# Gyeeta/gyeeta

Hardware: AMD Instinct MI355X
Metric: events/sec ingested + p50/p99 quantile error vs reference, 1→8 MI355X (higher is better)
Workload: dtype int64; 1 GPU; C3/C4: 10000 hosts x 1000 services, raw 24-B tcp_ipv4_resp_event_t stream, uniform over services, 1 window (ingest + window close) per step; service_keys_total=10000000, multi_level_windows=0, td_pend_cap=1920, td_pend_cap_is_library_default=False, exchange=none, exchange_requested=none, exchange_fallback=False

## Files before the change

gyeeta_amd/csrc/gys_kernels.hpp:

```cpp
#pragma once

#include "gys_device.hpp"

namespace gys {

#define GYS_HUGE_VALUE_BITS 20
#define GYS_HUGE_BINS (1u << GYS_HUGE_VALUE_BITS)
#define GYS_ROW_BITS 6
#define GYS_ROW_MASK 0x3Fu
#define GYS_ROW_V6 0x20u
#define GYS_BM_WORDS 32u
#define GYS_STAGED_WORD(tresp, cli_port) ((uint64_t)(((uint32_t)(tresp) << GYS_ROW_BITS) | ((uint32_t)(cli_port) & 0x1Fu)))
#define GYS_STAGED_WORD_FAM(tresp, cli_port, v6) ((uint32_t)(((uint32_t)(tresp) << GYS_ROW_BITS) | ((v6) ? GYS_ROW_V6 : 0u) | ((uint32_t)(cli_port) & 0x1Fu)))

enum { CTR_RESP_EVENTS = 0, CTR_RESP_DROP_RANGE, CTR_RESP_DROP_NOLISTENER, CTR_CONN_EVENTS, CTR_CONN_UNKNOWN, CTR_LSTATE_RECORDS,
       CTR_LSTATE_MISSED, CTR_LSTATE_ERRORS, CTR_LSTATE_DELETED, CTR_TD_MERGES, CTR_TD_MERGE_VALUES, CTR_ACTCONN_RECORDS, CTR_ACTCONN_REMOTE_LISTEN, CTR_ACTCONN_UNKNOWN,
       CTR_CONN_NEW, CTR_CONN_CLOSED, CTR_CONN_CLOSED_NO_NOTIFY, CTR_CONN_CLI_SIDE, CTR_RESP_RUN_OVERFLOW, CTR_NUM };

__global__ void k_table_set(DevTable t, const uint64_t *kv, uint32_t n)
{
	const uint32_t i = blockIdx.x * blockDim.x + threadIdx.x;
	if (i >= n) return;
	const uint64_t key = kv[2u * i];
	uint32_t h = get_uint64_hash(key) & t.mask;
// ... 1622 lines not shown
		for (uint32_t i = tid; i < GYS_IVL; i += NT) {
			s_icnt[i] = 0;
			s_imin[i] = 0xFFFFFFFFu;
			s_imax[i] = 0;
			s_clt[i] = 0;
		}
		if (tid < 16u) {
			s_fa[tid] = 0;
			s_fw[tid] = 0;
			s_fbm[tid] = 0;
			s_fbm[tid + 16u] = 0;
		}
		if (tid == 0) {
			s_fmm[0] = INT32_MAX;
			s_fmm[1] = INT32_MIN;
			s_fmm[2] = INT32_MIN;
		}
		__syncthreads();
		if (c0) {
			s_thr[pos0] = ceil_div_sum_cnt(sm0, c0);
			s_cpfx[pos0] = e0;
		}
		if (tid == 0) s_cpfx[nc] = nold;
		__syncthreads();
		{
			const uint32_t *pend = p.td_pend + (size_t)slot * p.pcap;
			int32_t lmin = INT32_MAX, lmax = INT32_MIN, wmax = INT32_MIN;
			for (uint32_t i = tid; i < m; i += NT) {
				const uint32_t word = i < ent.nbuf ? pend[i] : p.staged[run0 + (i - ent.nbuf)];
				const uint32_t uv = word >> GYS_ROW_BITS;
				uint32_t lo = 0;
#pragma unroll
				for (uint32_t step = GYS_NBP / 2; step >= 1u; step >>= 1)
					if (s_thr[lo + step - 1u] <= uv) lo += step;
				const uint32_t iv = lo + value_grid(uv);
				s_x[i] = (iv << 20) | uv;
				atomicAdd(&s_icnt[iv], 1u);
				atomicMin(&s_imin[iv], uv);
				atomicMax(&s_imax[iv], uv);
				atomicAdd(&s_clt[lo + 1], 1u);
				if (i >= nh) {
					const uint32_t b = resp_bucket((int64_t)uv);
					const unsigned long long one = GYS_PACK_ONE | (unsigned long long)uv;
					atomicAdd(&s_fa[b], one);
					lmin = min(lmin, (int32_t)uv);
					lmax = max(lmax, (int32_t)uv);
					if (i >= nwin0) {
						atomicAdd(&s_fw[b], one);
						const uint32_t r = word & GYS_ROW_MASK;
						atomicOr(&s_fbm[r >> 1], (1u << b) << ((r & 1u) * 16u));
						wmax = max(wmax, (int32_t)uv);
					}
				}
			}
			if (!query && m > nh) {
				lmin = wave_min_i32(lmin);
				lmax = wave_max_i32(lmax);
				wmax = wave_max_i32(wmax);
				if (lane == 0) {
					if (lmin != INT32_MAX) atomicMin(&s_fmm[0], lmin);
					if (lmax != INT32_MIN) atomicMax(&s_fmm[1], lmax);
					if (wmax != INT32_MIN) atomicMax(&s_fmm[2], wmax);
				}
			}
		}
		__syncthreads();
		if (wave == 0) {
			uint32_t t[5], gcl[5];
			uint32_t own = 0, gown = 0;
#pragma unroll
			for (int k = 0; k < 5; ++k) {
				t[k] = s_icnt[5u * lane + k];
				gcl[k] = s_clt[5u * lane + k];
				own += t[k];
				gown += gcl[k];
			}
			const uint32_t inc = wave_incl_scan_u32(own), ginc = wave_incl_scan_u32(gown);
			uint32_t ex = inc - own, gex = ginc - gown;
#pragma unroll
			for (int k = 0; k < 5; ++k) {
				s_ioff[5u * lane + k] = ex;
				s_icnt[5u * lane + k] = ex;
				ex += t[k];
				gex += gcl[k];
				s_clt[5u * lane + k] = gex;
			}
			if (lane == 63u) s_ioff[GYS_IVL] = inc;
		}
		__syncthreads();
		for (uint32_t i = tid; i < m; i += NT) {
			const uint32_t x = s_x[i];
			s_g[atomicAdd(&s_icnt[x >> 20], 1u)] = x;
		}
		__syncthreads();
		if (c0) {
			const uint64_t mid2 = 2ull * (e0 + (uint64_t)s_clt[pos0 + 1]) + (uint64_t)c0;
			uint32_t a = 0;
#pragma unroll
			for (uint32_t step = GYS_NBP / 2; step >= 1u; step >>= 1)
				if (mid2 >= s_T[a + step]) a += step;
			atomicAdd(&s_osum[a], (unsigned long long)sm0);
			atomicAdd(&s_ocnt[a], c0);
		}
		for (uint32_t e = tid; e < m; e += NT) {
			const uint32_t x = s_g[e];
			const uint32_t iv = x >> 20;
			uint32_t r = e;
			if (s_imin[iv] != s_imax[iv]) {
				const uint32_t gb = s_ioff[iv], ge = s_ioff[iv + 1];
				r = gb;
				for (uint32_t t = gb; t < ge; ++t) {
					const uint32_t y = s_g[t];
					r += (y < x || (y == x && t < e)) ? 1u : 0u;
				}
			}
			const uint64_t mid2 = 2ull * ((uint64_t)r + s_cpfx[iv - value_grid(x & 0xFFFFFu)]) + 1ull;
			uint32_t a = 0;
#pragma unroll
			for (uint32_t step = GYS_NBP / 2; step >= 1u; step >>= 1)
				if (mid2 >= s_T[a + step]) a += step;
			atomicAdd(&s_osum[a], (unsigned long long)(x & 0xFFFFFu));
			atomicAdd(&s_ocnt[a], 1u);
		}
		__syncthreads();
		if (tid < GYS_TD_NB) {
			int64_t *ws = query ? q.out_sum + (size_t)w * GYS_TD_NB : p.td_sum + (size_t)slot * GYS_TD_NB;
			uint32_t *wc = query ? q.out_cnt + (size_t)w * GYS_TD_NB : p.td_cnt + (size_t)slot * GYS_TD_NB;
			ws[tid] = (int64_t)s_osum[tid];
			wc[tid] = s_ocnt[tid];
		}
		if (!query) {
			const uint32_t n_all = m - nh, n_win = m > nwin0 ? m - nwin0 : 0u;
			if (tid < 16u && n_all) fold_records(p, slot, tid, mt.w != mt.z, s_fa[tid], s_fw[tid], n_all, n_win, s_fmm[1], s_fmm[2], s_fbm[tid], s_fbm[tid + 16u]);
			if (tid == 16u) {
				*(uint4 *)&p.td_meta[slot] = make_uint4(0u, 0u, mt.z, n_win ? mt.z : mt.w);
				p.td_cur[slot] = 0;
				if (n_all) {
					const int2 mm = p.td_minmax[slot];
					if (s_fmm[0] < mm.x || s_fmm[1] > mm.y) p.td_minmax[slot] = make_int2(min(mm.x, s_fmm[0]), max(mm.y, s_fmm[1]));
				}
			}
		}
		__syncthreads();
	}
}

#ifndef GYS_MB_SKIP
#define GYS_MB_SKIP 0
#endif
#define GYS_MB_EXACT 1024u
#define GYS_MB_BINS 2048u
#define GYS_MB_BPT 8u

__device__ __forceinline__ uint32_t mb_bin(uint32_t v)
{
	if (v < GYS_MB_EXACT) return v;
	const uint32_t msb = 31u - (uint32_t)__clz((int)v);
	return GYS_MB_EXACT + (msb - 10u) * 64u + ((v >> (msb - 6u)) & 63u);
}

struct MergeBP {
	DigestP d;
	const MergeEnt *list;
	const uint32_t *count;
	int64_t *out_sum;
	uint32_t *out_cnt;
	MergeEnt *slow_list;
	uint32_t *slow_count;
	const double *qs;
	uint32_t nq;
	double *qout;
};

__device__ __forceinline__ double td_quantile_dev(const uint32_t *c_cnt, const unsigned long long *c_sum, const uint32_t *c_wb, uint32_t nc, uint32_t N,
						  int32_t vmin, int32_t vmax, double q)
{
	if (!N) return 0.0;
	if (q < 0.0) q = 0.0;
	if (q > 1.0) q = 1.0;
	const double t = q * (double)N;
	uint32_t lo = 0, hi = nc;
	while (lo < hi) {
		const uint32_t mid = (lo + hi) >> 1;
		if (t < (double)c_wb[mid] + (double)c_cnt[mid] * 0.5) hi = mid; else lo = mid + 1;
	}
	double res;
	if (lo < nc) {
		const double mean = (double)(int64_t)c_sum[lo] / (double)c_cnt[lo];
		const double c = (double)c_wb[lo] + (double)c_cnt[lo] * 0.5;
		if (lo == 0) {
			const double l = (double)vmin;
			res = c <= 0.0 ? mean : l + (mean - l) * (t / c);
		} else {
			const double pm = (double)(int64_t)c_sum[lo - 1] / (double)c_cnt[lo - 1];
			const double pc = (double)c_wb[lo - 1] + (double)c_cnt[lo - 1] * 0.5;
			res = pm + (mean - pm) * ((t - pc) / (c - pc));
		}
	} else {
		const double pm = (double)(int64_t)c_sum[nc - 1] / (double)c_cnt[nc - 1];
		const double pc = (double)c_wb[nc - 1] + (double)c_cnt[nc - 1] * 0.5;
		const double h = (double)vmax, span = (double)N - pc;
		res = span <= 0.0 ? h : pm + (h - pm) * ((t - pc) / span);
	}
	return floor(res + 0.5);
}

#define GYS_MB_BIG_CAP 1024u
#ifndef GYS_MB_WAVES16
#define GYS_MB_WAVES16 5
#endif
template <bool SCAN, uint32_t VPT = 4u>
__global__ __launch_bounds__(256, (VPT == 16u ? GYS_MB_WAVES16 : 8)) void k_digest_bins(MergeBP q_arg)
{
#if defined(__HIP_DEVICE_COMPILE__)
	typedef const MergeBP __attribute__((address_space(4))) *KernargP;
	KernargP q_k = (KernargP)__builtin_amdgcn_kernarg_segment_ptr();
#define GYS_MB_Q_RELOAD() asm volatile("" : "+s"(q_k))
	const MergeBP &q = *(const MergeBP *)q_k;
#else
#define GYS_MB_Q_RELOAD() (void)0
	const MergeBP &q = q_arg;
#endif
	const DigestP &p = q.d;
	static_assert(VPT == 4u || VPT == 8u || VPT == 16u || VPT == 64u, "merges of 1024 / 2048 / 4096 values; 64: up to 16 384, streamed");
	constexpr bool STREAM = VPT > 16u;
	constexpr uint32_t RV = STREAM ? 8u : VPT;
	__shared__ __align__(16) uint32_t s_bin[GYS_MB_BINS];
	constexpr uint32_t BIG_CAP = GYS_MB_BIG_CAP;
	__shared__ uint32_t s_big[BIG_CAP];
	__shared__ uint32_t s_thr[GYS_NBP];
	__shared__ uint32_t s_cpfx[GYS_NBP + 1];
	__shared__ uint32_t s_T[GYS_NBP];
	__shared__ unsigned long long s_osum[GYS_TD_NB];
	__shared__ uint32_t s_ocnt[GYS_TD_NB];
	__shared__ unsigned long long s_oval[GYS_TD_NB];
	__shared__ unsigned long long s_fa[16], s_fw[16];
	__shared__ uint32_t s_fbm[GYS_BM_WORDS];
	__shared__ int32_t s_fmm[3];
	__shared__ uint32_t s_wv[4], s_ws[4], s_nbig;
	__shared__ uint64_t s_ww[4];
	const uint32_t nent = SCAN ? p.nsvc : *q.count;
	const bool query = SCAN || q.out_sum != nullptr;
	uint32_t bk_first = 0, bk_chg = GYS_MB_BPT;
	if (GYS_MB_BPT * threadIdx.x < GYS_MB_EXACT) {
		bk_first = resp_bucket((int64_t)(GYS_MB_BPT * threadIdx.x));
		for (uint32_t k = GYS_MB_BPT - 1u; k >= 1u; --k)
			if (resp_bucket((int64_t)(GYS_MB_BPT * threadIdx.x + k)) != bk_first) bk_chg = k;
	}

	for (uint32_t w = blockIdx.x; w < nent; w += gridDim.x) {
		uint32_t tid = threadIdx.x;
		GYS_OPAQUE_VGPR(tid);
		GYS_MB_Q_RELOAD();
		const uint32_t lane = tid & 63u, wave = tid >> 6;
		MergeEnt ent;
		if (SCAN) ent = MergeEnt{w, min(p.td_meta[w].npend, p.pend_cap), 0u, 0u};
		else ent = q.list[w];
		const uint32_t m = ent.nbuf + ent.mrun;
		if (m > 256u * VPT) continue;
		const uint32_t slot = ent.slot;
		const uint4 mt = *(const uint4 *)&p.td_meta[slot];
		const uint32_t nh = query ? m : (mt.y & 0xFFFFu), nw = mt.y >> 16;
		const uint32_t nh_mm = SCAN ? (mt.y & 0xFFFFu) : nh;
		const uint32_t nwin0 = max(nh, nw);
		const uint32_t run0 = ent.off_end - ent.mrun;
		uint32_t c0 = 0;
		int64_t sm0 = 0;
		if (tid < GYS_TD_NB) {
			c0 = p.td_cnt[(size_t)slot * GYS_TD_NB + tid];
			sm0 = p.td_sum[(size_t)slot * GYS_TD_NB + tid];
		}
		uint32_t wd[RV];
		const uint32_t *const pend = p.td_pend + (size_t)slot * p.pcap;
		{
#pragma unroll
			for (uint32_t k = 0; k < RV; ++k) {
				const uint32_t i = tid + 256u * k;
				wd[k] = 0;
				if (i < m) wd[k] = i < ent.nbuf ? pend[i] : p.staged[run0 + (i - ent.nbuf)];
			}
		}
		if (GYS_MB_SKIP & 32) {
			uint32_t x = c0 ^ (uint32_t)sm0;
#pragma unroll
			for (uint32_t k = 0; k < RV; ++k) x ^= wd[k];
			if (x == 0xDEADBEEFu) p.td_cur[slot] = 1;
			continue;
		}
		if (m == 0 && !SCAN) {
			if (query && tid < GYS_TD_NB) {
				q.out_sum[(size_t)w * GYS_TD_NB + tid] = sm0;
				q.out_cnt[(size_t)w * GYS_TD_NB + tid] = c0;
			}
			continue;
		}
#pragma unroll
		for (uint32_t k = 0; k < GYS_MB_BPT; ++k) s_bin[tid + 256u * k] = 0;
		s_thr[tid] = 0xFFFFFFFFu;
		if (tid < GYS_TD_NB) {
			s_osum[tid] = 0;
			s_ocnt[tid] = 0;
			s_oval[tid] = 0;
		}
		if (tid < 16u) {
			s_fa[tid] = 0;
			s_fw[tid] = 0;
			s_fbm[tid] = 0;
			s_fbm[tid + 16u] = 0;
		}
		if (tid == 0) {
			s_fmm[0] = INT32_MAX;
			s_fmm[1] = INT32_MIN;
			s_fmm[2] = INT32_MIN;
			s_nbig = 0;
		}
		const unsigned long long b0 = __ballot(c0 != 0);
		const uint64_t inc = wave_incl_scan_u64(c0);
		if (lane == 63u) s_ww[wave] = inc;
		if (lane == 0u) s_wv[wave] = (uint32_t)__popcll(b0);
		__syncthreads();
		uint32_t pbase = 0, nc = 0;
		uint64_t wbase = 0, nold64 = 0;
#pragma unroll
		for (uint32_t k = 0; k < 4u; ++k) {
			if (k < wave) {
				pbase += s_wv[k];
				wbase += s_ww[k];
			}
			nc += s_wv[k];
			nold64 += s_ww[k];
		}
		if (nold64 + (uint64_t)m >= (1ull << 31)) {
			if (tid == 0) q.slow_list[atomicAdd(q.slow_count, 1u)] = ent;
			__syncthreads();
			continue;
		}
		if (SCAN && m == 0) {
			if (tid < GYS_TD_NB) {
				s_osum[tid] = (unsigned long long)sm0;
				s_ocnt[tid] = c0;
			}
			__syncthreads();
		} else {
		const uint32_t pos0 = pbase + (uint32_t)__popcll(b0 & (lane ? (~0ull >> (64 - lane)) : 0ull));
		const uint32_t e0 = (uint32_t)(wbase + inc - c0), nold = (uint32_t)nold64;
		const uint32_t twoN = 2u * (nold + m);
		uint32_t thr = 0;
		if (c0) {
			thr = ceil_div_sum_cnt(sm0, c0);
			s_thr[pos0] = thr;
			s_cpfx[pos0] = e0;
			atomicAdd(&s_bin[mb_bin(thr)], 1u << 16);
		}
		if (tid == 0) s_cpfx[nc] = nold;
		s_T[tid] = (tid >= 1u && tid < GYS_TD_NB) ? (uint32_t)td_threshold(c_td_bnd[tid], (uint64_t)twoN) : (tid ? 0xFFFFFFFFu : 0u);
		const bool fold_scan = !query && nh == 0u;
		int32_t lmin = INT32_MAX, lmax = INT32_MIN, wmax = INT32_MIN;
		for (uint32_t cb = 0; cb < (STREAM ? m : 1u); cb += 256u * RV) {
		if (STREAM && cb) {
#pragma unroll
			for (uint32_t k = 0; k < RV; ++k) {
				const uint32_t i = cb + tid + 256u * k;
				wd[k] = 0;
				if (i < m) wd[k] = i < ent.nbuf ? pend[i] : p.staged[run0 + (i - ent.nbuf)];
			}
		}
#pragma unroll
		for (uint32_t k = 0; k < RV; ++k) {
			const uint32_t i = cb + tid + 256u * k;
			if (!(i >= m || (GYS_MB_SKIP & 4))) {
			const uint32_t uv = wd[k] >> GYS_ROW_BITS;
			atomicAdd(&s_bin[mb_bin(uv)], 1u);
			const bool big = uv >= GYS_MB_EXACT;
			if (big) {
				const uint32_t at = atomicAdd(&s_nbig, 1u);
				if (256u * VPT <= BIG_CAP || at < BIG_CAP) s_big[at] = STREAM ? uv : ((i << 20) | uv);
			}
			if (SCAN && i >= nh_mm) {
				lmin = min(lmin, (int32_t)uv);
				lmax = max(lmax, (int32_t)uv);
			}
			if (i >= nh) {
				lmin = min(lmin, (int32_t)uv);
				lmax = max(lmax, (int32_t)uv);
				const bool win = i >= nwin0;
				if (big || !fold_scan || win) {
					const uint32_t b = resp_bucket((int64_t)uv);
					const unsigned long long one = GYS_PACK_ONE | (unsigned long long)uv;
					if (big || !fold_scan) atomicAdd(&s_fa[b], one);
					if (win) {
						atomicAdd(&s_fw[b], one);
						const uint32_t r = wd[k] & GYS_ROW_MASK;
						atomicOr(&s_fbm[r >> 1], (1u << b) << ((r & 1u) * 16u));
						wmax = max(wmax, (int32_t)uv);
					}
				}
			}
			}
		}
		}
		if ((!query && m > nh) || (SCAN && m > nh_mm)) {
			lmin = wave_min_i32(lmin);
			lmax = wave_max_i32(lmax);
			wmax = wave_max_i32(wmax);
			if (lane == 0) {
				if (lmin != INT32_MAX) atomicMin(&s_fmm[0], lmin);
				if (lmax != INT32_MIN) atomicMax(&s_fmm[1], lmax);
				if (wmax != INT32_MIN) atomicMax(&s_fmm[2], wmax);
			}
		}
		__syncthreads();
		if (256u * VPT > BIG_CAP && s_nbig > BIG_CAP) {
			if (tid == 0) q.slow_list[atomicAdd(q.slow_count, 1u)] = ent;
			__syncthreads();
			continue;
		}
		if (!(GYS_MB_SKIP & 8)) {
			uint32_t bv[GYS_MB_BPT], own = 0;
			{
				const uint4 lo4 = ((const uint4 *)s_bin)[2u * tid], hi4 = ((const uint4 *)s_bin)[2u * tid + 1u];
				bv[0] = lo4.x; bv[1] = lo4.y; bv[2] = lo4.z; bv[3] = lo4.w;
				bv[4] = hi4.x; bv[5] = hi4.y; bv[6] = hi4.z; bv[7] = hi4.w;
			}
#pragma unroll
			for (uint32_t k = 0; k < GYS_MB_BPT; ++k) own += bv[k];
			const uint32_t sc = wave_incl_scan_u32(own);
			if (lane == 63u) s_ws[wave] = sc;
			__syncthreads();
			uint32_t run = sc - own;
#pragma unroll
			for (uint32_t k = 0; k < 3u; ++k)
				if (k < wave) run += s_ws[k];
			unsigned long long acc0 = 0, acc1 = 0;
#pragma unroll
			for (uint32_t k = 0; k < GYS_MB_BPT; ++k) {
				const uint32_t bin = GYS_MB_BPT * tid + k;
				const uint32_t raw = bv[k];
				bv[k] = (run & 0xFFFFu) | (((run >> 16) + (raw >> 16)) << 16);
				run += raw;
				const uint32_t cnt = raw & 0xFFFFu;
				const unsigned long long d = ((unsigned long long)(cnt << 8) << 32) | (unsigned long long)(cnt * bin);
				if (k < bk_chg) acc0 += d; else acc1 += d;
			}
			((uint4 *)s_bin)[2u * tid] = make_uint4(bv[0], bv[1], bv[2], bv[3]);
			((uint4 *)s_bin)[2u * tid + 1u] = make_uint4(bv[4], bv[5], bv[6], bv[7]);
			if (fold_scan && GYS_MB_BPT * tid < GYS_MB_EXACT) {
				if (acc0) atomicAdd(&s_fa[bk_first], acc0);
				if (acc1) atomicAdd(&s_fa[bk_first + 1u], acc1);
			}
		}
		__syncthreads();
		const uint32_t nbig = s_nbig;
		const bool has_old = c0 && !(GYS_MB_SKIP & 2);
		if (has_old) {
			uint32_t nb = s_bin[mb_bin(thr)] & 0xFFFFu;
			if (thr >= GYS_MB_EXACT) {
				const uint32_t sh = (31u - (uint32_t)__clz((int)thr)) - 6u;
				for (uint32_t j = 0; j < nbig; ++j) {
					const uint32_t u = s_big[j] & 0xFFFFFu;
					nb += ((u >> sh) == (thr >> sh) && u < thr) ? 1u : 0u;
				}
			}
			const uint32_t mid2 = 2u * (e0 + nb) + c0;
			uint32_t a = 0;
#pragma unroll
			for (uint32_t step = GYS_NBP / 2; step >= 1u; step >>= 1)
				if (mid2 >= s_T[a + step]) a += step;
			atomicAdd(&s_osum[a], (unsigned long long)sm0);
			atomicAdd(&s_ocnt[a], c0);
		}
#ifndef GYS_MB_GROUP
#define GYS_MB_GROUP 1u
#endif
		constexpr uint32_t MBG = SCAN ? 1u : GYS_MB_GROUP;
		const bool compact = MBG == 1u && nbig <= BIG_CAP / 2u;
		if (compact) {
			uint16_t *const s_ne = (uint16_t *)(s_big + BIG_CAP / 2u);
			const unsigned long long below = lane ? (~0ull >> (64 - lane)) : 0ull;
			uint32_t tw = 0, pos[4];
			bool ne[4];
#pragma unroll
			for (uint32_t k = 0; k < 4u; ++k) {
				const uint32_t b = tid + 256u * k;
				ne[k] = !(GYS_MB_SKIP & 1) && ((s_bin[b + 1u] ^ s_bin[b]) & 0xFFFFu) != 0u;
				const unsigned long long bal = __ballot(ne[k]);
				pos[k] = tw + (uint32_t)__popcll(bal & below);
				tw += (uint32_t)__popcll(bal);
			}
			if (lane == 0u) s_ws[wave] = tw;
			__syncthreads();
			uint32_t base = 0, n_ne = 0;
#pragma unroll
			for (uint32_t k = 0; k < 4u; ++k) {
				if (k < wave) base += s_ws[k];
				n_ne += s_ws[k];
			}
#pragma unroll
			for (uint32_t k = 0; k < 4u; ++k)
				if (ne[k]) s_ne[base + pos[k]] = (uint16_t)(tid + 256u * k);
			__syncthreads();
			for (uint32_t i = tid; i < n_ne; i += 256u) {
				const uint32_t b = s_ne[i];
				const uint32_t bw = s_bin[b];
				uint32_t rem = (s_bin[b + 1u] & 0xFFFFu) - (bw & 0xFFFFu), mid2 = 2u * ((bw & 0xFFFFu) + s_cpfx[bw >> 16]) + 1u, a = 0;
#pragma unroll
				for (uint32_t step = GYS_NBP / 2; step >= 1u; step >>= 1)
					if (mid2 >= s_T[a + step]) a += step;
				while (rem) {
					const uint32_t Tn = s_T[a + 1u];
					const uint32_t kk = min(rem, (Tn - mid2 + 1u) >> 1);
					atomicAdd(&s_oval[a], ((unsigned long long)kk << 40) | (unsigned long long)(kk * b));
					rem -= kk;
					mid2 += 2u * kk;
					++a;
				}
			}
		} else
#pragma unroll
		for (uint32_t k0 = 0; k0 < GYS_MB_EXACT / 256u; k0 += MBG) {
			uint32_t bq[MBG], cq[MBG], mq[MBG], aq[MBG], call = 0;
#pragma unroll
			for (uint32_t u = 0; u < MBG; ++u) {
				bq[u] = tid + 256u * (k0 + u);
				const uint32_t bw = s_bin[bq[u]];
				cq[u] = (GYS_MB_SKIP & 1) ? 0u : (s_bin[bq[u] + 1u] & 0xFFFFu) - (bw & 0xFFFFu);
				mq[u] = 2u * ((bw & 0xFFFFu) + s_cpfx[bw >> 16]) + 1u;
				aq[u] = 0;
				call |= cq[u];
			}
			if (!call) continue;
#pragma unroll
			for (uint32_t step = GYS_NBP / 2; step >= 1u; step >>= 1) {
				uint32_t tq[MBG];
#pragma unroll
				for (uint32_t u = 0; u < MBG; ++u) tq[u] = s_T[aq[u] + step];
#pragma unroll
				for (uint32_t u = 0; u < MBG; ++u)
					if (mq[u] >= tq[u]) aq[u] += step;
			}
#pragma unroll
			for (uint32_t u = 0; u < MBG; ++u) GYS_OPAQUE_VGPR(aq[u]);
#pragma unroll
			for (uint32_t u = 0; u < MBG; ++u) {
				uint32_t rem = cq[u], mid2 = mq[u], a = aq[u];
				const uint32_t b = bq[u];
				while (rem) {
					const uint32_t Tn = s_T[a + 1u];
					const uint32_t kk = min(rem, (Tn - mid2 + 1u) >> 1);
					atomicAdd(&s_oval[a], ((unsigned long long)kk << 40) | (unsigned long long)(kk * b));
					rem -= kk;
					mid2 += 2u * kk;
					++a;
				}
			}
		}
		for (uint32_t j = tid; j < ((GYS_MB_SKIP & 2) ? 0u : nbig); j += 256u) {
			const uint32_t me = s_big[j], uv = me & 0xFFFFFu, i = me >> 20;
			const uint32_t sh = (31u - (uint32_t)__clz((int)uv)) - 6u;
			uint32_t r = s_bin[mb_bin(uv)] & 0xFFFFu;
			for (uint32_t jj = 0; jj < nbig; ++jj) {
				const uint32_t e = s_big[jj], u = e & 0xFFFFFu;
				r += ((u >> sh) == (uv >> sh) && (u < uv || (u == uv && (STREAM ? jj < j : (e >> 20) < i)))) ? 1u : 0u;
			}
			uint32_t gap = 0;
#pragma unroll
			for (uint32_t step = GYS_NBP / 2; step >= 1u; step >>= 1)
				if (s_thr[gap + step - 1u] <= uv) gap += step;
			const uint32_t mid2 = 2u * (r + s_cpfx[gap]) + 1u;
			uint32_t a = 0;
#pragma unroll
			for (uint32_t step = GYS_NBP / 2; step >= 1u; step >>= 1)
				if (mid2 >= s_T[a + step]) a += step;
			atomicAdd(&s_oval[a], GYS_PACK_ONE | (unsigned long long)uv);
		}
		__syncthreads();
		if (tid < GYS_TD_NB) {
			const unsigned long long pv = s_oval[tid];
			s_osum[tid] += GYS_PACK_SUM(pv);
			s_ocnt[tid] += (uint32_t)(pv >> 40);
		}
		if (SCAN) __syncthreads();
		}
		if (SCAN) {
			const uint32_t oc = tid < GYS_TD_NB ? s_ocnt[tid] : 0u;
			const unsigned long long os = tid < GYS_TD_NB ? s_osum[tid] : 0ull;
			const unsigned long long ob = __ballot(oc != 0);
			const uint32_t sc = wave_incl_scan_u32(oc);
			if (lane == 63u) s_ws[wave] = sc;
			if (lane == 0u) s_wv[wave] = (uint32_t)__popcll(ob);
			__syncthreads();
			uint32_t pb = 0, wb = 0, ncq = 0, Nq = 0;
#pragma unroll
			for (uint32_t k = 0; k < 4u; ++k) {
				if (k < wave) {
					pb += s_wv[k];
					wb += s_ws[k];
				}
				ncq += s_wv[k];
				Nq += s_ws[k];
			}
			if (oc) {
				const uint32_t pos = pb + (uint32_t)__popcll(ob & (lane ? (~0ull >> (64 - lane)) : 0ull));
				s_thr[pos] = oc;
				s_cpfx[pos] = wb + sc - oc;
				s_osum[pos] = os;
			}
			__syncthreads();
			if (tid < q.nq) {
				const int2 mm = p.td_minmax[slot];
				q.qout[(size_t)slot * q.nq + tid] = td_quantile_dev(s_thr, s_osum, s_cpfx, ncq, Nq, min(mm.x, s_fmm[0]), max(mm.y, s_fmm[1]), q.qs[tid]);
			}
			__syncthreads();
			continue;
		}
		if (GYS_MB_SKIP & 16) {
			if (tid == 208u && !query) {
				*(uint4 *)&p.td_meta[slot] = make_uint4(0u, 0u, mt.z, mt.w);
				p.td_cur[slot] = 0;
			}
			__syncthreads();
			continue;
		}
		if (tid < GYS_TD_NB) {
			int64_t *ws = query ? q.out_sum + (size_t)w * GYS_TD_NB : p.td_sum + (size_t)slot * GYS_TD_NB;
			uint32_t *wc = query ? q.out_cnt + (size_t)w * GYS_TD_NB : p.td_cnt + (size_t)slot * GYS_TD_NB;
			ws[tid] = (int64_t)s_osum[tid];
			wc[tid] = s_ocnt[tid];
		}
		if (!query) {
			const uint32_t n_all = m - nh, n_win = m > nwin0 ? m - nwin0 : 0u;
			if (tid >= 192u && tid < 208u && n_all)
				fold_records(p, slot, tid - 192u, mt.w != mt.z, s_fa[tid - 192u], s_fw[tid - 192u], n_all, n_win, s_fmm[1], s_fmm[2], s_fbm[tid - 192u], s_fbm[tid - 176u]);
			if (tid == 208u) {
				*(uint4 *)&p.td_meta[slot] = make_uint4(0u, 0u, mt.z, n_win ? mt.z : mt.w);
				p.td_cur[slot] = 0;
				if (n_all) {
					const int2 mm = p.td_minmax[slot];
					if (s_fmm[0] < mm.x || s_fmm[1] > mm.y) p.td_minmax[slot] = make_int2(min(mm.x, s_fmm[0]), max(mm.y, s_fmm[1]));
				}
			}
		}
		__syncthreads();
	}
}

struct HugeP {
	DigestP d;
	const MergeEnt *huge_list;
	const uint32_t *huge_count;
	uint32_t *scratch;
};

__global__ __launch_bounds__(256) void k_digest_huge(HugeP p)
{
	__shared__ int64_t s_csum[GYS_TD_NB];
	__shared__ uint32_t s_ccnt[GYS_TD_NB];
	__shared__ uint64_t s_cpfx[GYS_TD_NB + 1];
	__shared__ uint64_t s_T[GYS_TD_NB + 1];
	__shared__ unsigned long long s_osum[GYS_TD_NB];
	__shared__ unsigned long long s_ocnt[GYS_TD_NB];
	__shared__ uint32_t s_part[256];
	__shared__ uint32_t s_wave[4];
	__shared__ unsigned long long s_ha[32], s_hw[32];
	__shared__ uint32_t s_bm[GYS_BM_WORDS];
	__shared__ uint32_t s_nc;
	__shared__ int32_t s_min, s_max, s_wmax;
	uint32_t *bins = p.scratch + (size_t)blockIdx.x * GYS_HUGE_BINS;
	const uint32_t nh_list = *p.huge_count;
	const uint32_t BPT = GYS_HUGE_BINS / 256u;

	for (uint32_t w = blockIdx.x; w < nh_list; w += gridDim.x) {
		const MergeEnt ent = p.huge_list[w];
		const uint32_t slot = ent.slot;
		const uint32_t m = ent.mrun, npend = ent.nbuf;
		const uint32_t start = ent.off_end - m;
		const uint4 mt = *(const uint4 *)&p.d.td_meta[slot];
		const uint32_t nh = mt.y & 0xFFFFu, nw = mt.y >> 16;
		const uint32_t nwin0 = max(nh, nw);
		const uint32_t *pend = p.d.td_pend + (size_t)slot * p.d.pcap;
		for (uint32_t i = threadIdx.x; i < GYS_HUGE_BINS / 4u; i += 256u) ((uint4 *)bins)[i] = make_uint4(0, 0, 0, 0);
		if (threadIdx.x < GYS_TD_NB) {
			s_osum[threadIdx.x] = 0;
			s_ocnt[threadIdx.x] = 0;
		}
		if (threadIdx.x < 32u) {
			s_ha[threadIdx.x] = 0;
			s_hw[threadIdx.x] = 0;
		}
		if (threadIdx.x >= 160u && threadIdx.x < 160u + GYS_BM_WORDS) s_bm[threadIdx.x - 160u] = 0;
		if (threadIdx.x == 0) {
			const int64_t *gs = p.d.td_sum + (size_t)slot * GYS_TD_NB;
			const uint32_t *gc = p.d.td_cnt + (size_t)slot * GYS_TD_NB;
			uint32_t nc = 0;
			uint64_t run = 0;
			for (uint32_t j = 0; j < GYS_TD_NB; ++j) {
				if (gc[j]) {
					s_csum[nc] = gs[j];
					s_ccnt[nc] = gc[j];
					s_cpfx[nc] = run;
					run += gc[j];
					nc++;
				}
			}
			s_cpfx[nc] = run;
			s_nc = nc;
			s_min = INT32_MAX;
			s_max = INT32_MIN;
			s_wmax = INT32_MIN;
		}
		__syncthreads();
		const uint32_t nc = s_nc;
		const uint64_t nold = s_cpfx[nc];
		const uint64_t twoN = 2ull * (nold + (uint64_t)m + (uint64_t)npend);
		if (threadIdx.x >= 1 && threadIdx.x < GYS_TD_NB) s_T[threadIdx.x] = td_threshold(c_td_bnd[threadIdx.x], twoN);
		if (threadIdx.x == 0) s_T[GYS_TD_NB] = ~0ull;
// ... 1848 lines not shown
```

gyeeta_amd/csrc/gys_rollup.hpp:

```cpp
#pragma once

namespace gys {

#define GYS_RB_FINE 1920u
#define GYS_RB_HEAVY 1024u
#define GYS_RB_HDR (2u * GYS_MB_BINS + 2u)
#define GYS_RB_MARK (GYS_RB_HDR + 1u)
#define GYS_RB_FCNT (GYS_RB_MARK + GYS_MB_BINS / 8u)
#define GYS_RB_FSUM (GYS_RB_FCNT + GYS_RB_FINE)
#define GYS_RB_STRIDE (GYS_RB_FSUM + GYS_RB_FINE)
#ifndef GYS_RB_NT
#define GYS_RB_NT 1024u
#endif
#ifndef GYS_RB_AHEAD
#define GYS_RB_AHEAD 2u
#endif
#ifndef GYS_RB_WAVES
#define GYS_RB_WAVES 8
#endif
#ifndef GYS_RB_VC
#define GYS_RB_VC 4096u
#endif

struct RollupChunk {
	uint32_t group, m0, m1, pad;
};

struct RollupP {
	DigestP d;
	const RollupChunk *chunks;
	uint32_t nchunks;
	const uint32_t *members;
	int kind;
	const gys_tdigest_slab *in;
	unsigned long long *bins;
	gys_tdigest_slab *out;
	uint32_t ngroups;
};

__global__ __launch_bounds__(256) void k_rollup_init(unsigned long long *bins, uint32_t ngroups)
{
	const size_t n = (size_t)ngroups * (GYS_RB_HDR + 1u);
	for (size_t i = (size_t)blockIdx.x * 256u + threadIdx.x; i < n; i += (size_t)gridDim.x * 256u) {
		const uint32_t k = (uint32_t)(i % (GYS_RB_HDR + 1u));
		bins[i / (GYS_RB_HDR + 1u) * GYS_RB_STRIDE + k] =
			k == 2u * GYS_MB_BINS ? (unsigned long long)(long long)INT32_MAX : k == 2u * GYS_MB_BINS + 1u ? (unsigned long long)(long long)INT32_MIN : 0ull;
	}
}

__device__ __forceinline__ uint32_t ceil_div_wide(uint64_t sum, uint64_t cnt)
{
	if ((int64_t)sum <= 0) return 0u;
	const double dq = (double)sum / (double)cnt;
	if (dq >= 4294967040.0) return 0xFFFFFFFFu;
	uint64_t f = (uint64_t)dq;
	int64_t r = (int64_t)(sum - f * cnt);
	if (r < 0) {
		f--;
		r += (int64_t)cnt;
	} else if ((uint64_t)r >= cnt) {
		f++;
		r -= (int64_t)cnt;
	}
	f += r != 0;
	return f > 0xFFFFFFFFull ? 0xFFFFFFFFu : (uint32_t)f;
}

__device__ __forceinline__ uint32_t rb_bin(uint32_t v) { return mb_bin(v < (1u << 26) ? v : (1u << 26) - 1u); }

#if GYS_RB_WAVES
__global__ __launch_bounds__(GYS_RB_NT, GYS_RB_WAVES) void k_rollup_accum(RollupP q)
#else
__global__ __launch_bounds__(GYS_RB_NT) void k_rollup_accum(RollupP q)
#endif
{
	const DigestP &p = q.d;
	__shared__ unsigned long long s_cnt[GYS_MB_BINS], s_sum[GYS_MB_BINS];
	__shared__ uint32_t s_vc[GYS_RB_VC];
	__shared__ long long s_mm[2];
	const uint32_t tid = threadIdx.x, lane = tid & 63u, wave = tid >> 6;
	constexpr uint32_t NW = GYS_RB_NT / 64u;

	for (uint32_t c = blockIdx.x; c < q.nchunks; c += gridDim.x) {
		for (uint32_t k = tid; k < GYS_MB_BINS; k += GYS_RB_NT) {
			s_cnt[k] = 0;
			s_sum[k] = 0;
		}
		for (uint32_t k = tid; k < GYS_RB_VC; k += GYS_RB_NT) s_vc[k] = 0;
		if (tid == 0) {
			s_mm[0] = INT32_MAX;
			s_mm[1] = INT32_MIN;
		}
		__syncthreads();
		const RollupChunk ck = q.chunks[c];
		long long mmin = INT32_MAX, mmax = INT32_MIN;
		int32_t lmin = INT32_MAX, lmax = INT32_MIN;
		uint32_t mem_n = 0, npend_n = 0;
		if (ck.m0 + wave < ck.m1) {
			mem_n = q.members[ck.m0 + wave];
			if (q.kind == 0) npend_n = min(p.td_meta[mem_n].npend, p.pend_cap);
		}
		for (uint32_t mi = ck.m0 + wave; mi < ck.m1; mi += NW) {
			const uint32_t mem = mem_n, npend = npend_n;
			if (mi + NW < ck.m1) {
				mem_n = q.members[mi + NW];
				if (q.kind == 0) npend_n = min(p.td_meta[mem_n].npend, p.pend_cap);
			}
			const uint32_t *pend = p.td_pend + (size_t)mem * p.pcap;
			const bool quads = q.kind == 0 && (p.pcap & 3u) == 0u;
			uint4 va[GYS_RB_AHEAD];
#pragma unroll
			for (uint32_t k = 0; k < GYS_RB_AHEAD; ++k) {
				va[k] = make_uint4(0, 0, 0, 0);
				if (quads && 4u * lane + 256u * k < npend) va[k] = ((const uint4 *)pend)[lane + 64u * k];
			}
			bool any = false;
#pragma unroll
			for (uint32_t k = 0; k < (GYS_TD_NB + 63u) / 64u; ++k) {
				const uint32_t j = lane + 64u * k;
				uint64_t cn = 0, sm = 0;
				if (j < GYS_TD_NB) {
					if (q.kind == 0) {
						cn = p.td_cnt[(size_t)mem * GYS_TD_NB + j];
						sm = (uint64_t)p.td_sum[(size_t)mem * GYS_TD_NB + j];
					} else {
						cn = q.in[mem].cnt[j];
						sm = (uint64_t)q.in[mem].sum[j];
					}
				}
				if (cn) {
					const uint32_t b = rb_bin(ceil_div_wide(sm, cn));
					atomicAdd(&s_cnt[b], (unsigned long long)cn);
					atomicAdd(&s_sum[b], (unsigned long long)sm);
				}
				any |= __ballot(cn != 0) != 0ull;
			}
			if (any && lane == 0) {
				long long vmn, vmx;
				if (q.kind == 0) {
					const int2 mm = p.td_minmax[mem];
					vmn = mm.x;
					vmx = mm.y;
				} else {
					vmn = q.in[mem].vmin;
					vmx = q.in[mem].vmax;
				}
				mmin = vmn < mmin ? vmn : mmin;
				mmax = vmx > mmax ? vmx : mmax;
			}
			if (q.kind != 0) continue;
			auto one = [&](uint32_t word) {
				if (word < (GYS_RB_VC << GYS_ROW_BITS)) {
					atomicAdd((uint32_t *)((char *)s_vc + ((word >> (GYS_ROW_BITS - 2u)) & ~3u)), 1u);
				} else {
					const uint32_t uv = word >> GYS_ROW_BITS, b = rb_bin(uv);
					atomicAdd(&s_cnt[b], 1ull);
					atomicAdd(&s_sum[b], (unsigned long long)uv);
					lmin = min(lmin, (int32_t)uv);
					lmax = max(lmax, (int32_t)uv);
				}
			};
			auto quad = [&](const uint4 w4, uint32_t i) {
				if (i + 3u < npend) {
					one(w4.x);
					one(w4.y);
					one(w4.z);
					one(w4.w);
				} else {
					if (i < npend) one(w4.x);
					if (i + 1u < npend) one(w4.y);
					if (i + 2u < npend) one(w4.z);
				}
			};
			if (quads) {
#pragma unroll
				for (uint32_t k = 0; k < GYS_RB_AHEAD; ++k) quad(va[k], 4u * lane + 256u * k);
#pragma unroll 2
				for (uint32_t i = 4u * lane + 256u * GYS_RB_AHEAD; i < npend; i += 256u) quad(((const uint4 *)pend)[i >> 2], i);
			} else {
#pragma unroll 4
				for (uint32_t i = lane; i < npend; i += 64u) one(pend[i]);
			}
		}
		__syncthreads();
		for (uint32_t k = tid; k < GYS_RB_VC; k += GYS_RB_NT) {
			const uint32_t vc = s_vc[k];
			if (!vc) continue;
			lmin = min(lmin, (int32_t)k);
			lmax = max(lmax, (int32_t)k);
			if (k >= GYS_MB_EXACT) {
				const uint32_t b = rb_bin(k);
				atomicAdd(&s_cnt[b], (unsigned long long)vc);
				atomicAdd(&s_sum[b], (unsigned long long)vc * k);
			}
		}
		lmin = wave_min_i32(lmin);
		lmax = wave_max_i32(lmax);
		if (lane == 0) {
			mmin = (long long)lmin < mmin ? (long long)lmin : mmin;
			mmax = (long long)lmax > mmax ? (long long)lmax : mmax;
			if (mmin != INT32_MAX) atomicMin(&s_mm[0], mmin);
			if (mmax != INT32_MIN) atomicMax(&s_mm[1], mmax);
		}
		__syncthreads();
		unsigned long long *gb = q.bins + (size_t)ck.group * GYS_RB_STRIDE;
		for (uint32_t k = tid; k < GYS_MB_BINS; k += GYS_RB_NT) {
			unsigned long long cn = s_cnt[k], sm = s_sum[k];
			if (k < GYS_MB_EXACT) {
				const uint32_t vc = s_vc[k];
				cn += vc;
				sm += (unsigned long long)vc * k;
			}
			if (cn) {
				atomicAdd(&gb[k], cn);
				atomicAdd(&gb[GYS_MB_BINS + k], sm);
			}
		}
		if (tid == 0) {
			if (s_mm[0] != INT32_MAX) atomicMin((long long *)&gb[2u * GYS_MB_BINS], s_mm[0]);
			if (s_mm[1] != INT32_MIN) atomicMax((long long *)&gb[2u * GYS_MB_BINS + 1u], s_mm[1]);
		}
		__syncthreads();
	}
}

__device__ __forceinline__ uint64_t mul_div_floor(uint64_t s, uint64_t k, uint64_t w)
{
	const uint64_t hi = __umul64hi(s, k), lo = s * k;
	if (!hi) return lo / w;
	uint64_t qt = 0, rem = hi;
	for (int i = 63; i >= 0; --i) {
		const bool carry = (rem >> 63) != 0;
		rem = (rem << 1) | ((lo >> i) & 1ull);
		qt <<= 1;
		if (carry || rem >= w) {
			rem -= w;
			qt |= 1ull;
		}
	}
	return qt;
}

__device__ __forceinline__ uint32_t cluster_of_u64(const uint64_t *T, uint64_t mid2)
{
	uint32_t a = 0;
#pragma unroll
	for (uint32_t step = GYS_NBP / 2; step >= 1u; step >>= 1)
		if (mid2 >= T[a + step]) a += step;
	return a;
}

__device__ __forceinline__ uint32_t rb_ncell(uint32_t b, uint32_t per) { return min(per, 1u << (4u + (b - GYS_MB_EXACT) / 64u)); }
__device__ __forceinline__ uint32_t rb_cell(uint32_t v, uint32_t b, uint32_t per)
{
	const uint32_t sh = 4u + (b - GYS_MB_EXACT) / 64u, lo = (64u + ((b - GYS_MB_EXACT) & 63u)) << sh;
	return ((v - lo) * rb_ncell(b, per)) >> sh;
}

__global__ __launch_bounds__(256) void k_rollup_mark(RollupP q)
{
	__shared__ uint64_t s_T[GYS_NBP];
	__shared__ uint64_t s_ww[4];
	__shared__ uint32_t s_wm[4];
	const uint32_t tid = threadIdx.x, lane = tid & 63u, wave = tid >> 6;

	for (uint32_t g = blockIdx.x; g < q.ngroups; g += gridDim.x) {
		unsigned long long *gb = q.bins + (size_t)g * GYS_RB_STRIDE;
		uint64_t cn[GYS_MB_BPT], own = 0;
#pragma unroll
		for (uint32_t k = 0; k < GYS_MB_BPT; ++k) {
			cn[k] = gb[GYS_MB_BPT * tid + k];
			own += cn[k];
		}
		const uint64_t inc = wave_incl_scan_u64(own);
		if (lane == 63u) s_ww[wave] = inc;
		__syncthreads();
		uint64_t W = inc - own, N = 0;
#pragma unroll
		for (uint32_t k = 0; k < 4u; ++k) {
			if (k < wave) W += s_ww[k];
			N += s_ww[k];
		}
		s_T[tid] = (tid >= 1u && tid < GYS_TD_NB) ? td_threshold(c_td_bnd[tid], 2ull * N) : (tid ? ~0ull : 0ull);
		__syncthreads();
		uint32_t mk = 0;
#pragma unroll
		for (uint32_t k = 0; k < GYS_MB_BPT; ++k) {
			const uint64_t w = cn[k];
			if (GYS_MB_BPT * tid + k >= GYS_MB_EXACT && w > N / GYS_RB_HEAVY &&
			    cluster_of_u64(s_T, 2ull * W + 1ull) != cluster_of_u64(s_T, 2ull * (W + w - 1ull) + 1ull))
				mk |= 1u << k;
			W += w;
		}
		const uint32_t nm = (uint32_t)__popc(mk), minc = wave_incl_scan_u32(nm);
		if (lane == 63u) s_wm[wave] = minc;
		__syncthreads();
		uint32_t idx = minc - nm, total = 0;
#pragma unroll
		for (uint32_t k = 0; k < 4u; ++k) {
			if (k < wave) idx += s_wm[k];
			total += s_wm[k];
		}
		unsigned long long word = 0;
#pragma unroll
		for (uint32_t k = 0; k < GYS_MB_BPT; ++k)
			if (mk & (1u << k)) word |= (unsigned long long)(++idx) << (8u * k);
		gb[GYS_RB_MARK + tid] = word;
		const uint32_t per = total ? GYS_RB_FINE / total : 0u;
		if (tid == 0) gb[GYS_RB_HDR] = (unsigned long long)total | ((unsigned long long)per << 32);
		for (uint32_t k = tid; k < total * per; k += 256u) {
			gb[GYS_RB_FCNT + k] = 0ull;
			gb[GYS_RB_FSUM + k] = 0ull;
		}
		__syncthreads();
	}
}

__global__ __launch_bounds__(GYS_RB_NT) void k_rollup_refine(RollupP q)
{
	const DigestP &p = q.d;
	__shared__ unsigned long long f_cnt[GYS_RB_FINE], f_sum[GYS_RB_FINE];
	__shared__ unsigned long long s_mark[GYS_MB_BINS / 8u];
	const uint32_t tid = threadIdx.x, lane = tid & 63u, wave = tid >> 6;
	constexpr uint32_t NW = GYS_RB_NT / 64u;

	for (uint32_t c = blockIdx.x; c < q.nchunks; c += gridDim.x) {
		const RollupChunk ck = q.chunks[c];
		unsigned long long *gb = q.bins + (size_t)ck.group * GYS_RB_STRIDE;
		const unsigned long long hdr = gb[GYS_RB_HDR];
		const uint32_t per = (uint32_t)(hdr >> 32), ncell = (uint32_t)hdr * per;
		if (!ncell) continue;
		for (uint32_t k = tid; k < GYS_MB_BINS / 8u; k += GYS_RB_NT) s_mark[k] = gb[GYS_RB_MARK + k];
		for (uint32_t k = tid; k < ncell; k += GYS_RB_NT) {
			f_cnt[k] = 0;
			f_sum[k] = 0;
		}
		__syncthreads();
		const uint8_t *mark = (const uint8_t *)s_mark;
		auto put = [&](uint32_t v, uint64_t cn, uint64_t sm) {
			v = min(v, (1u << 26) - 1u);
			const uint32_t b = mb_bin(v), m = mark[b];
			if (m) {
				const uint32_t cell = (m - 1u) * per + rb_cell(v, b, per);
				atomicAdd(&f_cnt[cell], (unsigned long long)cn);
				atomicAdd(&f_sum[cell], (unsigned long long)sm);
			}
		};
		for (uint32_t mi = ck.m0 + wave; mi < ck.m1; mi += NW) {
			const uint32_t mem = q.members[mi];
#pragma unroll
			for (uint32_t k = 0; k < (GYS_TD_NB + 63u) / 64u; ++k) {
				const uint32_t j = lane + 64u * k;
				uint64_t cn = 0, sm = 0;
				if (j < GYS_TD_NB) {
					if (q.kind == 0) {
						cn = p.td_cnt[(size_t)mem * GYS_TD_NB + j];
						sm = (uint64_t)p.td_sum[(size_t)mem * GYS_TD_NB + j];
					} else {
						cn = q.in[mem].cnt[j];
						sm = (uint64_t)q.in[mem].sum[j];
					}
				}
				if (cn) put(ceil_div_wide(sm, cn), cn, sm);
			}
			if (q.kind != 0) continue;
			const uint32_t npend = min(p.td_meta[mem].npend, p.pend_cap);
			const uint32_t *pend = p.td_pend + (size_t)mem * p.pcap;
			for (uint32_t i = lane; i < npend; i += 64u) {
				const uint32_t word = pend[i];
				if (word >= (GYS_MB_EXACT << GYS_ROW_BITS)) put(word >> GYS_ROW_BITS, 1ull, word >> GYS_ROW_BITS);
			}
		}
		__syncthreads();
		for (uint32_t k = tid; k < ncell; k += GYS_RB_NT) {
			if (f_cnt[k]) {
				atomicAdd(&gb[GYS_RB_FCNT + k], f_cnt[k]);
				atomicAdd(&gb[GYS_RB_FSUM + k], f_sum[k]);
			}
		}
		__syncthreads();
	}
}

__global__ __launch_bounds__(256) void k_rollup_cluster(RollupP q)
{
	__shared__ uint64_t s_T[GYS_NBP];
	__shared__ unsigned long long o_sum[GYS_NBP], o_cnt[GYS_NBP];
	__shared__ unsigned long long f_cnt[GYS_RB_FINE], f_sum[GYS_RB_FINE];
	__shared__ uint64_t s_ww[4];
	const uint32_t tid = threadIdx.x, lane = tid & 63u, wave = tid >> 6;

	for (uint32_t g = blockIdx.x; g < q.ngroups; g += gridDim.x) {
		const unsigned long long *gb = q.bins + (size_t)g * GYS_RB_STRIDE;
		uint64_t cn[GYS_MB_BPT], sm[GYS_MB_BPT], own = 0;
#pragma unroll
		for (uint32_t k = 0; k < GYS_MB_BPT; ++k) {
			cn[k] = gb[GYS_MB_BPT * tid + k];
			sm[k] = gb[GYS_MB_BINS + GYS_MB_BPT * tid + k];
			own += cn[k];
		}
		const unsigned long long hdr = gb[GYS_RB_HDR];
		const uint32_t per = (uint32_t)(hdr >> 32), ncell = (uint32_t)hdr * per;
		const unsigned long long mword = ncell ? gb[GYS_RB_MARK + tid] : 0ull;
		for (uint32_t k = tid; k < ncell; k += 256u) {
			f_cnt[k] = gb[GYS_RB_FCNT + k];
			f_sum[k] = gb[GYS_RB_FSUM + k];
		}
		const uint64_t inc = wave_incl_scan_u64(own);
		if (lane == 63u) s_ww[wave] = inc;
		o_sum[tid] = 0;
		o_cnt[tid] = 0;
		__syncthreads();
		uint64_t W = inc - own, N = 0;
#pragma unroll
		for (uint32_t k = 0; k < 4u; ++k) {
			if (k < wave) W += s_ww[k];
			N += s_ww[k];
		}
		s_T[tid] = (tid >= 1u && tid < GYS_TD_NB) ? td_threshold(c_td_bnd[tid], 2ull * N) : (tid ? ~0ull : 0ull);
		__syncthreads();
		auto unit = [&](uint64_t w, uint64_t s) {
			if (!w) return;
			uint32_t a = cluster_of_u64(s_T, 2ull * W + 1ull);
			uint64_t r = 0, given = 0;
			while (r < w) {
				const uint64_t Tn = s_T[a + 1u];
				uint64_t r1 = w;
				if (Tn != ~0ull) {
					const uint64_t x = Tn > 2ull * W ? (Tn - 2ull * W) >> 1 : 0ull;
					r1 = x < w ? x : w;
				}
				if (r1 > r) {
					const uint64_t upto = r1 == w ? s : mul_div_floor(s, r1, w);
					atomicAdd(&o_sum[a], (unsigned long long)(upto - given));
					atomicAdd(&o_cnt[a], (unsigned long long)(r1 - r));
					given = upto;
					r = r1;
				}
				++a;
			}
			W += w;
		};
		if (N) {
#pragma unroll 1
			for (uint32_t k = 0; k < GYS_MB_BPT; ++k) {
				const uint32_t m = (uint32_t)(mword >> (8u * k)) & 255u;
				if (!m) {
					unit(cn[k], sm[k]);
					continue;
				}
				const uint32_t c0 = (m - 1u) * per, c1 = c0 + rb_ncell(GYS_MB_BPT * tid + k, per);
#pragma unroll 1
				for (uint32_t c = c0; c < c1; ++c) unit(f_cnt[c], f_sum[c]);
			}
		}
		__syncthreads();
		if (tid < GYS_TD_NB) {
			q.out[g].sum[tid] = (int64_t)o_sum[tid];
			q.out[g].cnt[tid] = o_cnt[tid];
		}
		if (tid == 0) {
			q.out[g].vmin = (int64_t)gb[2u * GYS_MB_BINS];
			q.out[g].vmax = (int64_t)gb[2u * GYS_MB_BINS + 1u];
		}
		__syncthreads();
	}
}

}
```

Baseline: 65.70 billion events/s.

## Fold nonempty-bin compaction into prefix scan and vectorize big-value rank loops

Builds the compacted list of nonempty exact bins inside the existing prefix-scan pass, using a per-wave count scan. This removes the separate ballot pass and its two barriers. Computes the log bin with a float bit-cast instead of clz and keeps the clz version for rollup, whose values can exceed the float-exact range. The big-value rank loops now use range-subtract comparisons and uint4 LDS reads, with ties broken by a rotated index key. The compaction now keys on nonzero counts rather than prefix differences and reuses s_wv, so there is correctness risk if those don't match exactly.

```diff
diff --git a/gyeeta_amd/csrc/gys_kernels.hpp b/gyeeta_amd/csrc/gys_kernels.hpp
--- a/gyeeta_amd/csrc/gys_kernels.hpp
+++ b/gyeeta_amd/csrc/gys_kernels.hpp
@@ -1798,11 +1798,17 @@
 #define GYS_MB_BINS 2048u
 #define GYS_MB_BPT 8u
 
-__device__ __forceinline__ uint32_t mb_bin(uint32_t v)
+__device__ __forceinline__ uint32_t mb_bin_clz(uint32_t v)
 {
 	if (v < GYS_MB_EXACT) return v;
 	const uint32_t msb = 31u - (uint32_t)__clz((int)v);
 	return GYS_MB_EXACT + (msb - 10u) * 64u + ((v >> (msb - 6u)) & 63u);
+}
+
+__device__ __forceinline__ uint32_t mb_bin(uint32_t v)
+{
+	if (v < GYS_MB_EXACT) return v;
+	return (__builtin_bit_cast(uint32_t, (float)v) >> 17) - 7744u;
 }
 
 struct MergeBP {
@@ -1873,7 +1879,7 @@
 	constexpr uint32_t RV = STREAM ? 8u : VPT;
 	__shared__ __align__(16) uint32_t s_bin[GYS_MB_BINS];
 	constexpr uint32_t BIG_CAP = GYS_MB_BIG_CAP;
-	__shared__ uint32_t s_big[BIG_CAP];
+	__shared__ __align__(16) uint32_t s_big[BIG_CAP];
 	__shared__ uint32_t s_thr[GYS_NBP];
 	__shared__ uint32_t s_cpfx[GYS_NBP + 1];
 	__shared__ uint32_t s_T[GYS_NBP];
@@ -2071,12 +2077,31 @@
 #pragma unroll
 			for (uint32_t k = 0; k < GYS_MB_BPT; ++k) own += bv[k];
 			const uint32_t sc = wave_incl_scan_u32(own);
-			if (lane == 63u) s_ws[wave] = sc;
+			uint32_t ne_own = 0, ne_sc = 0;
+			if (GYS_MB_BPT * 64u * wave < GYS_MB_EXACT) {
+#pragma unroll
+				for (uint32_t k = 0; k < GYS_MB_BPT; ++k) ne_own += (bv[k] & 0xFFFFu) ? 1u : 0u;
+				ne_sc = wave_incl_scan_u32(ne_own);
+			}
+			if (lane == 63u) {
+				s_ws[wave] = sc;
+				s_wv[wave] = ne_sc;
+			}
 			__syncthreads();
 			uint32_t run = sc - own;
 #pragma unroll
 			for (uint32_t k = 0; k < 3u; ++k)
 				if (k < wave) run += s_ws[k];
+			if (GYS_MB_BPT * 64u * wave < GYS_MB_EXACT && s_nbig <= BIG_CAP / 2u) {
+				uint16_t *const s_ne = (uint16_t *)(s_big + BIG_CAP / 2u);
+				uint32_t at = ne_sc - ne_own;
+#pragma unroll
+				for (uint32_t k = 0; k < (GYS_MB_EXACT / (GYS_MB_BPT * 64u)) - 1u; ++k)
+					if (k < wave) at += s_wv[k];
+#pragma unroll
+				for (uint32_t k = 0; k < GYS_MB_BPT; ++k)
+					if (bv[k] & 0xFFFFu) s_ne[at++] = (uint16_t)(GYS_MB_BPT * tid + k);
+			}
 			unsigned long long acc0 = 0, acc1 = 0;
 #pragma unroll
 			for (uint32_t k = 0; k < GYS_MB_BPT; ++k) {
@@ -2102,10 +2127,14 @@
 			uint32_t nb = s_bin[mb_bin(thr)] & 0xFFFFu;
 			if (thr >= GYS_MB_EXACT) {
 				const uint32_t sh = (31u - (uint32_t)__clz((int)thr)) - 6u;
-				for (uint32_t j = 0; j < nbig; ++j) {
-					const uint32_t u = s_big[j] & 0xFFFFFu;
-					nb += ((u >> sh) == (thr >> sh) && u < thr) ? 1u : 0u;
-				}
+				const uint32_t lo = (thr >> sh) << sh, span = thr - lo;
+				const uint32_t n4 = nbig & ~3u;
+				for (uint32_t j = 0; j < n4; j += 4u) {
+					const uint4 e4 = *(const uint4 *)&s_big[j];
+					nb += ((e4.x & 0xFFFFFu) - lo < span ? 1u : 0u) + ((e4.y & 0xFFFFFu) - lo < span ? 1u : 0u) + ((e4.z & 0xFFFFFu) - lo < span ? 1u : 0u) +
+					      ((e4.w & 0xFFFFFu) - lo < span ? 1u : 0u);
+				}
+				for (uint32_t j = n4; j < nbig; ++j) nb += (s_big[j] & 0xFFFFFu) - lo < span ? 1u : 0u;
 			}
 			const uint32_t mid2 = 2u * (e0 + nb) + c0;
 			uint32_t a = 0;
@@ -2121,30 +2150,12 @@
 		constexpr uint32_t MBG = SCAN ? 1u : GYS_MB_GROUP;
 		const bool compact = MBG == 1u && nbig <= BIG_CAP / 2u;
 		if (compact) {
-			uint16_t *const s_ne = (uint16_t *)(s_big + BIG_CAP / 2u);
-			const unsigned long long below = lane ? (~0ull >> (64 - lane)) : 0ull;
-			uint32_t tw = 0, pos[4];
-			bool ne[4];
-#pragma unroll
-			for (uint32_t k = 0; k < 4u; ++k) {
-				const uint32_t b = tid + 256u * k;
-				ne[k] = !(GYS_MB_SKIP & 1) && ((s_bin[b + 1u] ^ s_bin[b]) & 0xFFFFu) != 0u;
-				const unsigned long long bal = __ballot(ne[k]);
-				pos[k] = tw + (uint32_t)__popcll(bal & below);
-				tw += (uint32_t)__popcll(bal);
-			}
-			if (lane == 0u) s_ws[wave] = tw;
-			__syncthreads();
-			uint32_t base = 0, n_ne = 0;
-#pragma unroll
-			for (uint32_t k = 0; k < 4u; ++k) {
-				if (k < wave) base += s_ws[k];
-				n_ne += s_ws[k];
-			}
-#pragma unroll
-			for (uint32_t k = 0; k < 4u; ++k)
-				if (ne[k]) s_ne[base + pos[k]] = (uint16_t)(tid + 256u * k);
-			__syncthreads();
+			const uint16_t *const s_ne = (const uint16_t *)(s_big + BIG_CAP / 2u);
+			uint32_t n_ne = 0;
+			if (!(GYS_MB_SKIP & (1 | 8))) {
+#pragma unroll
+				for (uint32_t k = 0; k < GYS_MB_EXACT / (GYS_MB_BPT * 64u); ++k) n_ne += s_wv[k];
+			}
 			for (uint32_t i = tid; i < n_ne; i += 256u) {
 				const uint32_t b = s_ne[i];
 				const uint32_t bw = s_bin[b];
@@ -2201,12 +2212,26 @@
 			}
 		}
 		for (uint32_t j = tid; j < ((GYS_MB_SKIP & 2) ? 0u : nbig); j += 256u) {
-			const uint32_t me = s_big[j], uv = me & 0xFFFFFu, i = me >> 20;
+			const uint32_t me = s_big[j], uv = me & 0xFFFFFu;
 			const uint32_t sh = (31u - (uint32_t)__clz((int)uv)) - 6u;
 			uint32_t r = s_bin[mb_bin(uv)] & 0xFFFFu;
-			for (uint32_t jj = 0; jj < nbig; ++jj) {
-				const uint32_t e = s_big[jj], u = e & 0xFFFFFu;
-				r += ((u >> sh) == (uv >> sh) && (u < uv || (u == uv && (STREAM ? jj < j : (e >> 20) < i)))) ? 1u : 0u;
+			if (STREAM) {
+				for (uint32_t jj = 0; jj < nbig; ++jj) {
+					const uint32_t e = s_big[jj], u = e & 0xFFFFFu;
+					r += ((u >> sh) == (uv >> sh) && (u < uv || (u == uv && jj < j))) ? 1u : 0u;
+				}
+			} else {
+				const uint32_t base = ((uv >> sh) << sh) << 12, span = ((me << 12) | (me >> 20)) - base;
+				const uint32_t n4 = nbig & ~3u;
+				for (uint32_t jj = 0; jj < n4; jj += 4u) {
+					const uint4 e4 = *(const uint4 *)&s_big[jj];
+					r += ((((e4.x << 12) | (e4.x >> 20)) - base < span) ? 1u : 0u) + ((((e4.y << 12) | (e4.y >> 20)) - base < span) ? 1u : 0u) +
+					     ((((e4.z << 12) | (e4.z >> 20)) - base < span) ? 1u : 0u) + ((((e4.w << 12) | (e4.w >> 20)) - base < span) ? 1u : 0u);
+				}
+				for (uint32_t jj = n4; jj < nbig; ++jj) {
+					const uint32_t e = s_big[jj];
+					r += (((e << 12) | (e >> 20)) - base < span) ? 1u : 0u;
+				}
 			}
 			uint32_t gap = 0;
 #pragma unroll
diff --git a/gyeeta_amd/csrc/gys_rollup.hpp b/gyeeta_amd/csrc/gys_rollup.hpp
--- a/gyeeta_amd/csrc/gys_rollup.hpp
+++ b/gyeeta_amd/csrc/gys_rollup.hpp
@@ -66,7 +66,7 @@
 	return f > 0xFFFFFFFFull ? 0xFFFFFFFFu : (uint32_t)f;
 }
 
-__device__ __forceinline__ uint32_t rb_bin(uint32_t v) { return mb_bin(v < (1u << 26) ? v : (1u << 26) - 1u); }
+__device__ __forceinline__ uint32_t rb_bin(uint32_t v) { return mb_bin_clz(v < (1u << 26) ? v : (1u << 26) - 1u); }
 
 #if GYS_RB_WAVES
 __global__ __launch_bounds__(GYS_RB_NT, GYS_RB_WAVES) void k_rollup_accum(RollupP q)
@@ -339,7 +339,7 @@
 		const uint8_t *mark = (const uint8_t *)s_mark;
 		auto put = [&](uint32_t v, uint64_t cn, uint64_t sm) {
 			v = min(v, (1u << 26) - 1u);
-			const uint32_t b = mb_bin(v), m = mark[b];
+			const uint32_t b = mb_bin_clz(v), m = mark[b];
 			if (m) {
 				const uint32_t cell = (m - 1u) * per + rb_cell(v, b, per);
 				atomicAdd(&f_cnt[cell], (unsigned long long)cn);
```

Result: faster. 70.96 billion events/s, median of 6 (+8.0%).
